# featureform/embeddinghub

Hardware: NVIDIA H100
Metric: k-NN queries/s (higher is better)
Workload: dtype f32

## Files before the change

embeddinghub_b200/csrc/walk.cuh:

```cuda
#pragma once
#include <cuda_bf16.h>

#include <type_traits>

#include "common.cuh"

namespace ehb {

struct GraphView {
  const float* vecs;
  const uint32_t* links0;
  const uint32_t* up_off;
  const uint32_t* links_up;
  const uint64_t* labels;
  const uint8_t* deleted;
  uint32_t n, dim, dpad, M, M0, entry;
  int32_t max_level;
  int32_t metric;
  const __nv_bfloat16* vecs16;
  const int8_t* codes8;
  const float4* terms8;
};

struct WalkCfg {
  uint32_t lcap;
  uint32_t hash_size;
  uint32_t G;
  uint32_t NG;
  uint32_t staged;
  uint32_t dense;
  uint32_t prefetch;
  uint32_t dcap;
};

constexpr uint32_t kMaxSinks = 16;
struct ResultSink {
  uint64_t* labels[kMaxSinks];
  float* dists[kMaxSinks];
  uint32_t* flags[kMaxSinks];
  uint32_t* slice_count;
  uint32_t n, qs, epoch;
  uint64_t* keys;
};

__host__ __device__ inline uint32_t align_up(uint32_t x, uint32_t a) { return (x + a - 1) / a * a; }

constexpr uint32_t kPadDims[] = {32, 64, 128, 256, 384, 512, 768, 1024, 1536, 2048};
constexpr uint32_t kNumPadDims = sizeof(kPadDims) / sizeof(kPadDims[0]);
__host__ __device__ constexpr int row_lpv(uint32_t row_bytes) { return row_bytes > 1024 ? 32 : 8; }
__host__ __device__ constexpr int row_nq(uint32_t dpad, uint32_t row_bytes) {
  return (int)(dpad / (4u * (uint32_t)row_lpv(row_bytes)));
}
constexpr int kpl_for(uint32_t ef) { return ef <= 64 ? 2 : (ef <= 128 ? 4 : (ef <= 256 ? 8 : 16)); }

inline uint32_t pad_dim(uint32_t dim) {
  for (uint32_t d : kPadDims)
    if (dim <= d) return d;
  return 0;
}

template <uint32_t MaxDpad = 2048, uint32_t I = 0, class F>
cudaError_t with_dpad(uint32_t dpad, F&& f) {
  if constexpr (I == kNumPadDims || kPadDims[I] > MaxDpad)
    return cudaErrorInvalidValue;
  else
    return dpad == kPadDims[I] ? f(std::integral_constant<uint32_t, kPadDims[I]>{})
                               : with_dpad<MaxDpad, I + 1>(dpad, f);
}

__host__ __device__ constexpr bool screen_shape(int LPV, int NQ) { return LPV == 32 && NQ <= 12; }

__host__ __device__ inline uint32_t warp_smem_bytes(const WalkCfg& c, uint32_t vbytes) {
  uint32_t b = 0;
  b += align_up(c.lcap * 8u, 128);
  b += align_up(c.hash_size * 4u, 128);
  b += 128;
  b += 128;
  b += 128;
  b += align_up(c.dcap * 8u, 128);
  b += c.staged ? align_up(c.G * c.NG * vbytes, 128) : 0u;
  return b;
}

struct WarpCtx {
  uint64_t* keys;
  uint32_t* hash;
  uint32_t* cand_id;
  float* cand_dist;
  uint64_t* mbar;
  uint32_t* dq_hi;
  uint32_t* dq_id;
  float* stage;
  uint32_t lcap, hsize, G, NG, dpad, vbytes, dcap, prefetch;
  uint32_t phases;
  uint32_t cnt;
  uint32_t lane;
};

__device__ __forceinline__ void ctx_init(WarpCtx& c, unsigned char* base, const WalkCfg& cfg, uint32_t dpad,
                                         uint32_t esize = 4u) {
  c.lane = lane_id();
  c.lcap = cfg.lcap;
  c.G = cfg.G;
  c.NG = cfg.NG;
  c.dpad = dpad;
  c.vbytes = dpad * esize;
  c.hsize = cfg.hash_size;
  unsigned char* p = base;
  c.keys = (uint64_t*)p;
  p += align_up(cfg.lcap * 8u, 128);
  c.hash = (uint32_t*)p;
  p += align_up(cfg.hash_size * 4u, 128);
  c.cand_id = (uint32_t*)p;
  p += 128;
  c.cand_dist = (float*)p;
  p += 128;
  c.mbar = (uint64_t*)p;
  p += 128;
  c.dcap = cfg.dcap;
  c.prefetch = cfg.prefetch;
  c.dq_hi = (uint32_t*)p;
  c.dq_id = c.dq_hi + cfg.dcap;
  p += align_up(cfg.dcap * 8u, 128);
  c.stage = (float*)p;
  c.phases = 0;
  c.cnt = 0;
  if (cfg.staged) {
    if (c.lane < cfg.NG) mbar_init(&c.mbar[c.lane], 1);
    fence_mbar_init();
  }
  __syncwarp();
}

__device__ __forceinline__ void hash_clear(WarpCtx& c) {
  uint4* h4 = (uint4*)c.hash;
  uint32_t n4 = c.hsize >> 2;
  for (uint32_t i = c.lane; i < n4; i += 32) h4[i] = make_uint4(kInvalid, kInvalid, kInvalid, kInvalid);
  __syncwarp();
}

__device__ __forceinline__ bool hash_insert(WarpCtx& c, uint32_t id, uint32_t& overflow) {
  uint32_t h = __umulhi(id * 0x9E3779B1u, c.hsize);
#pragma unroll 1
  for (int probe = 0; probe < 8; ++probe) {
    uint32_t old = atomicCAS(&c.hash[h], kInvalid, id);
    if (old == kInvalid) return true;
    if (old == id) return false;
    h = h + 1u == c.hsize ? 0u : h + 1u;
  }
  overflow = 1;
  return true;
}

template <class RowT, int NQ, int W = (std::is_same<RowT, __nv_bfloat16>::value && NQ > 1) ? 8 : 4>
struct LaneChunks {
  static_assert(W == 4 || (W == 8 && std::is_same<RowT, __nv_bfloat16>::value), "no such chunk");
  using T = std::conditional_t<std::is_same<RowT, float>::value, float4,
                               std::conditional_t<std::is_same<RowT, int8_t>::value, uint32_t,
                                                  std::conditional_t<W == 8, uint4, uint2>>>;
  static constexpr int V = W / 4;
  static constexpr int N = NQ / V;
};
__device__ __forceinline__ float4 ld_chunk(const float4* p) { return ld_nc_f4(p); }
__device__ __forceinline__ uint4 ld_chunk(const uint4* p) { return ld_nc_u4(p); }
__device__ __forceinline__ uint2 ld_chunk(const uint2* p) { return ld_nc_u2(p); }
__device__ __forceinline__ float4 bf16x4_to_f4(uint32_t a, uint32_t b) {
  return make_float4(__uint_as_float(a << 16), __uint_as_float(a & 0xFFFF0000u), __uint_as_float(b << 16),
                     __uint_as_float(b & 0xFFFF0000u));
}
__device__ __forceinline__ void widen(const float4& v, float4* x) { x[0] = v; }
__device__ __forceinline__ void widen(const uint4& v, float4* x) {
  x[0] = bf16x4_to_f4(v.x, v.y);
  x[1] = bf16x4_to_f4(v.z, v.w);
}
__device__ __forceinline__ void widen(const uint2& v, float4* x) { x[0] = bf16x4_to_f4(v.x, v.y); }
__device__ __forceinline__ void widen(const uint32_t& v, float4* x) {
  const uint32_t u = v ^ 0x80808080u;
  x[0] = make_float4(__uint_as_float(__byte_perm(u, 0x4B000000u, 0x7540)) - 8388736.0f,
                     __uint_as_float(__byte_perm(u, 0x4B000000u, 0x7541)) - 8388736.0f,
                     __uint_as_float(__byte_perm(u, 0x4B000000u, 0x7542)) - 8388736.0f,
                     __uint_as_float(__byte_perm(u, 0x4B000000u, 0x7543)) - 8388736.0f);
}

template <int LPV, int NQ, class RowT = float>
__device__ __forceinline__ void load_query_regs(float4 (&qr)[NQ], const float* __restrict__ src, uint32_t dim,
                                                uint32_t lane) {
  constexpr int V = LaneChunks<RowT, NQ>::V;
  uint32_t sub = lane % LPV;
#pragma unroll
  for (int t = 0; t < NQ; ++t) {
    uint32_t e = (sub + LPV * (t / V)) * 4u * V + 4u * (t % V);
    float4 v;
    v.x = e + 0 < dim ? src[e + 0] : 0.f;
    v.y = e + 1 < dim ? src[e + 1] : 0.f;
    v.z = e + 2 < dim ? src[e + 2] : 0.f;
    v.w = e + 3 < dim ? src[e + 3] : 0.f;
    qr[t] = v;
  }
}
template <int LPV, int NQ, class RowT, class C = LaneChunks<RowT, NQ>>
__device__ __forceinline__ void load_vec_regs(typename C::T (&r)[C::N], const RowT* __restrict__ row,
                                              uint32_t lane) {
  const typename C::T* p = (const typename C::T*)row + (lane % LPV);
#pragma unroll
  for (int t = 0; t < C::N; ++t) r[t] = p[LPV * t];
}

template <int NQ>
__device__ __forceinline__ float partial_dist(const float4 (&v)[NQ], const float4 (&qr)[NQ], int metric) {
  float a0 = 0.f, a1 = 0.f, a2 = 0.f, a3 = 0.f;
  if (metric == 0) {
#pragma unroll
    for (int t = 0; t < NQ; ++t) {
      float dx = qr[t].x - v[t].x, dy = qr[t].y - v[t].y, dz = qr[t].z - v[t].z, dw = qr[t].w - v[t].w;
      a0 = fmaf(dx, dx, a0);
      a1 = fmaf(dy, dy, a1);
      a2 = fmaf(dz, dz, a2);
      a3 = fmaf(dw, dw, a3);
    }
  } else {
#pragma unroll
    for (int t = 0; t < NQ; ++t) {
      a0 = fmaf(qr[t].x, v[t].x, a0);
      a1 = fmaf(qr[t].y, v[t].y, a1);
      a2 = fmaf(qr[t].z, v[t].z, a2);
      a3 = fmaf(qr[t].w, v[t].w, a3);
    }
  }
  return (a0 + a1) + (a2 + a3);
}
template <int LPV>
__device__ __forceinline__ float group_reduce(float acc) {
#pragma unroll
  for (int o = LPV / 2; o > 0; o >>= 1) acc += __shfl_xor_sync(0xffffffffu, acc, o);
  return acc;
}

template <int NQ, class RowT, class C = LaneChunks<RowT, NQ>>
__device__ __forceinline__ float chunk_dist(const typename C::T (&v)[C::N], const float4 (&qr)[NQ], int metric) {
  float4 x[NQ];
#pragma unroll
  for (int j = 0; j < C::N; ++j) widen(v[j], x + j * C::V);
  return partial_dist<NQ>(x, qr, metric);
}
template <class RowT>
__device__ __forceinline__ const RowT* walk_rows(const GraphView& g) {
  if constexpr (std::is_same<RowT, float>::value)
    return g.vecs;
  else
    return g.vecs16;
}

__host__ __device__ constexpr int eval_u(int N, int UDIV) {
  return ((N <= 2 ? 8 : (N <= 4 ? 4 : 2)) / UDIV) > 0 ? (N <= 2 ? 8 : (N <= 4 ? 4 : 2)) / UDIV : 1;
}
template <int NQ, int U = eval_u(NQ, 1), class RowT = float>
__device__ __forceinline__ void eval_direct(WarpCtx& c, const RowT* __restrict__ rows, const float4 (&qr)[NQ],
                                            uint32_t m, int metric) {
  using C = LaneChunks<RowT, NQ>;
  const uint32_t sub = c.lane & 7u, grp = c.lane >> 3;
  __syncwarp();
#pragma unroll 1
  for (uint32_t j0 = 0; j0 < m; j0 += 4 * U) {
    typename C::T v[U][C::N];
#pragma unroll
    for (int u = 0; u < U; ++u) {
      if (j0 + 4u * u < m) {
        uint32_t j = min(j0 + 4u * u + grp, m - 1u);
        const typename C::T* p = (const typename C::T*)(rows + (size_t)c.cand_id[j] * c.dpad) + sub;
#pragma unroll
        for (int t = 0; t < C::N; ++t) v[u][t] = ld_chunk(p + 8 * t);
      }
    }
#pragma unroll
    for (int u = 0; u < U; ++u) {
      if (j0 + 4u * u < m) {
        uint32_t j = j0 + 4u * u + grp;
        float acc = group_reduce<8>(chunk_dist<NQ, RowT>(v[u], qr, metric));
        if (sub == 0 && j < m) c.cand_dist[j] = metric == 0 ? acc : 1.0f - acc;
      }
    }
  }
  __syncwarp();
}

template <class RowT>
__device__ __forceinline__ void issue_rows(WarpCtx& c, const RowT* __restrict__ vecs, uint32_t r, uint32_t m,
                                           uint32_t G, uint32_t vbytes) {
  uint32_t buf = r % c.NG;
  uint32_t first = r * G;
  uint32_t cnt = min(G, m - first);
  if (c.lane == 0) mbar_arrive_expect_tx(&c.mbar[buf], cnt * vbytes);
  __syncwarp();
  if (c.lane < cnt) {
    uint32_t id = c.cand_id[first + c.lane];
    bulk_g2s((RowT*)c.stage + (size_t)(buf * G + c.lane) * c.dpad, vecs + (size_t)id * c.dpad, vbytes, &c.mbar[buf]);
  }
}
template <class RowT>
__device__ __forceinline__ void issue_group(WarpCtx& c, const RowT* __restrict__ vecs, uint32_t r, uint32_t m) {
  issue_rows(c, vecs, r, m, c.G, c.vbytes);
}
template <int NQ, class RowT>
__device__ __forceinline__ void eval_staged(WarpCtx& c, const RowT* __restrict__ vecs, const float4 (&qr)[NQ],
                                            uint32_t m, int metric) {
  const uint32_t rounds = (m + c.G - 1) / c.G;
  const uint32_t pre = min(rounds, c.NG);
  for (uint32_t r = 0; r < pre; ++r) issue_group(c, vecs, r, m);
#pragma unroll 1
  for (uint32_t r = 0; r < rounds; ++r) {
    uint32_t buf = r % c.NG;
    mbar_wait(&c.mbar[buf], (c.phases >> buf) & 1u);
    c.phases ^= (1u << buf);
    uint32_t first = r * c.G;
    uint32_t cnt = min(c.G, m - first);
#pragma unroll 1
    for (uint32_t v0 = 0; v0 < cnt; v0 += 4) {
      float acc[4];
#pragma unroll
      for (int i = 0; i < 4; ++i) {
        uint32_t v = min(v0 + (uint32_t)i, cnt - 1u);
        typename LaneChunks<RowT, NQ>::T x[LaneChunks<RowT, NQ>::N];
        load_vec_regs<32, NQ>(x, (const RowT*)c.stage + (size_t)(buf * c.G + v) * c.dpad, c.lane);
        acc[i] = chunk_dist<NQ, RowT>(x, qr, metric);
      }
#pragma unroll
      for (int o = 16; o > 0; o >>= 1) {
#pragma unroll
        for (int i = 0; i < 4; ++i) acc[i] += __shfl_xor_sync(0xffffffffu, acc[i], o);
      }
      if (c.lane < 4 && v0 + c.lane < cnt) {
        float a = c.lane == 0 ? acc[0] : (c.lane == 1 ? acc[1] : (c.lane == 2 ? acc[2] : acc[3]));
        c.cand_dist[first + v0 + c.lane] = metric == 0 ? a : 1.0f - a;
      }
    }
    __syncwarp();
    if (r + c.NG < rounds) {
      fence_proxy_async();
      issue_group(c, vecs, r + c.NG, m);
    }
  }
  __syncwarp();
}

template <int LPV, int NQ, int UDIV = 1, class RowT = float>
__device__ __forceinline__ void eval_candidates(WarpCtx& c, const RowT* __restrict__ vecs, const float4 (&qr)[NQ],
                                                uint32_t m, int metric) {
  if (LPV == 8)
    eval_direct<NQ, eval_u(LaneChunks<RowT, NQ>::N, UDIV)>(c, vecs, qr, m, metric);
  else
    eval_staged<NQ>(c, vecs, qr, m, metric);
}

struct ScreenQuery {
  float l1, l2, a;
};
__device__ __forceinline__ ScreenQuery* screen_query(const WarpCtx& c) { return (ScreenQuery*)(c.mbar + 8); }
template <int NQ>
__device__ __forceinline__ uint32_t screen_staged(WarpCtx& c, const GraphView& g, const float4 (&qr)[NQ], uint32_t m,
                                                  uint32_t worst_hi, uint32_t& unsure) {
  using C = LaneChunks<int8_t, NQ>;
  constexpr int SV = 4;
  const uint32_t G = min(4u * c.G, 32u), vbytes = c.dpad;
  const uint32_t rounds = (m + G - 1) / G;
  const uint32_t pre = min(rounds, c.NG);
  const bool in = c.lane < m;
  fence_proxy_async();
  for (uint32_t r = 0; r < pre; ++r) issue_rows(c, g.codes8, r, m, G, vbytes);
  if (in) prefetch_l2(g.terms8 + c.cand_id[c.lane]);
#pragma unroll 1
  for (uint32_t r = 0; r < rounds; ++r) {
    uint32_t buf = r % c.NG;
    mbar_wait(&c.mbar[buf], (c.phases >> buf) & 1u);
    c.phases ^= (1u << buf);
    uint32_t first = r * G;
    uint32_t cnt = min(G, m - first);
#pragma unroll 1
    for (uint32_t v0 = 0; v0 < cnt; v0 += SV) {
      float e[SV];
#pragma unroll
      for (int i = 0; i < SV; ++i) {
        uint32_t v = min(v0 + (uint32_t)i, cnt - 1u);
        const typename C::T* s4 = (const typename C::T*)((const int8_t*)c.stage + (size_t)(buf * G + v) * c.dpad) +
                                  c.lane;
        float4 x[NQ];
#pragma unroll
        for (int t = 0; t < C::N; ++t) widen(s4[32 * t], x + t);
        e[i] = partial_dist<NQ>(x, qr, 1);
      }
#pragma unroll
      for (int o = 16; o > 0; o >>= 1) {
#pragma unroll
        for (int i = 0; i < SV; ++i) e[i] += __shfl_xor_sync(0xffffffffu, e[i], o);
      }
      if (c.lane < (uint32_t)SV && v0 + c.lane < cnt) {
        float ea = e[0];
#pragma unroll
        for (int i = 1; i < SV; ++i)
          if (c.lane == (uint32_t)i) ea = e[i];
        c.cand_dist[first + v0 + c.lane] = ea;
      }
    }
    __syncwarp();
    if (r + c.NG < rounds) {
      fence_proxy_async();
      issue_rows(c, g.codes8, r + c.NG, m, G, vbytes);
    }
  }
  __syncwarp();
  float L = 0.f;
  const uint32_t id = in ? c.cand_id[c.lane] : kInvalid;
  if (in) {
    const float4 tm = ld_nc_f4(g.terms8 + id);
    const ScreenQuery sq = *screen_query(c);
    const float e = (float)c.dpad * 0x1p-24f;
    const float gam = __fdiv_ru(e, 1.0f - e), as = __fmul_ru((float)c.dpad, 0x1p-118f);
    const float se = __fmul_ru(tm.x, c.cand_dist[c.lane]);
    float mg = __fmul_ru(__fmul_ru(gam, sq.l2), __fmaf_ru(2.0f, tm.w, tm.z));
    mg = __fadd_ru(mg, fminf(__fmul_ru(sq.l1, tm.y), __fmul_ru(sq.l2, tm.z)));
    mg = __fadd_ru(mg, __fmaf_ru(tm.x, as, sq.a));
    L = __fsub_rd(__fsub_rd(1.0f, se), mg);
  }
  const bool keep = in && !(isfinite(L) && f2ord(L) >= worst_hi);
  const uint32_t mask = __ballot_sync(0xffffffffu, keep);
  const uint32_t pos = __popc(mask & lanemask_lt());
  __syncwarp();
  if (keep) c.cand_id[pos] = id;
  if (unsure) unsure = __reduce_or_sync(0xffffffffu, (keep && ((unsure >> c.lane) & 1u)) ? (1u << pos) : 0u);
  fence_proxy_async();
  __syncwarp();
  return __popc(mask);
}

template <int KPL>
struct UList {
  uint32_t hi[KPL];
  uint32_t id[KPL];
};
template <int KPL>
__device__ __forceinline__ void ul_clear(UList<KPL>& u, uint32_t ef, uint32_t lane) {
#pragma unroll
  for (int s = 0; s < KPL; ++s) {
    u.hi[s] = ((uint32_t)s * 32u + lane) < ef ? 0xFFFFFFFFu : 0u;
    u.id[s] = kInvalid;
  }
}
template <int KPL>
__device__ __forceinline__ uint32_t ul_worst(const UList<KPL>& u) {
  uint32_t m = u.hi[0];
#pragma unroll
  for (int s = 1; s < KPL; ++s) m = max(m, u.hi[s]);
  return __reduce_max_sync(0xffffffffu, m);
}
template <int KPL>
__device__ __forceinline__ void ul_insert(UList<KPL>& u, uint32_t hi, uint32_t id, uint32_t ef, uint32_t& cnt,
                                          uint32_t& worst_hi, uint32_t lane) {
  bool done = false;
  if (cnt < ef) {
#pragma unroll
    for (int s = 0; s < KPL; ++s) {
      if (!done) {
        uint32_t b = __ballot_sync(0xffffffffu, u.id[s] == kInvalid && u.hi[s] == 0xFFFFFFFFu);
        if (b) {
          if ((int)lane == __ffs(b) - 1) u.hi[s] = hi, u.id[s] = id;
          done = true;
        }
      }
    }
    cnt++;
    if (cnt == ef) worst_hi = ul_worst<KPL>(u);
  } else {
#pragma unroll
    for (int s = 0; s < KPL; ++s) {
      if (!done) {
        uint32_t b = __ballot_sync(0xffffffffu, u.hi[s] == worst_hi && u.id[s] != kInvalid);
        if (b) {
          if ((int)lane == __ffs(b) - 1) u.hi[s] = hi, u.id[s] = id;
          done = true;
        }
      }
    }
    worst_hi = ul_worst<KPL>(u);
  }
}
template <int KPL>
__device__ __forceinline__ uint32_t ul_min_unexpanded(UList<KPL>& u, bool mark, uint32_t lane) {
  uint32_t m = 0xFFFFFFFFu;
#pragma unroll
  for (int s = 0; s < KPL; ++s)
    if (!(u.id[s] & kExpandedFlag)) m = min(m, u.hi[s]);
  m = __reduce_min_sync(0xffffffffu, m);
  uint32_t node = kInvalid;
  bool done = false;
#pragma unroll
  for (int s = 0; s < KPL; ++s) {
    if (!done) {
      uint32_t b = __ballot_sync(0xffffffffu, !(u.id[s] & kExpandedFlag) && u.hi[s] == m);
      if (b) {
        int l = __ffs(b) - 1;
        node = __shfl_sync(0xffffffffu, u.id[s], l);
        if (mark && (int)lane == l) u.id[s] |= kExpandedFlag;
        done = true;
      }
    }
  }
  return node;
}
template <int KPL>
__device__ __forceinline__ uint32_t ul_min_unexpanded_hi(const UList<KPL>& u) {
  uint32_t m = 0xFFFFFFFFu;
#pragma unroll
  for (int s = 0; s < KPL; ++s)
    if (!(u.id[s] & kExpandedFlag)) m = min(m, u.hi[s]);
  return __reduce_min_sync(0xffffffffu, m);
}
template <int KPL>
__device__ __forceinline__ bool ul_contains(const UList<KPL>& u, uint32_t id) {
  bool hit = false;
#pragma unroll
  for (int s = 0; s < KPL; ++s) hit |= u.id[s] != kInvalid && (u.id[s] & kIdMask) == id;
  return __any_sync(0xffffffffu, hit);
}
template <int KPL>
__device__ __forceinline__ uint64_t ul_extract_min(UList<KPL>& u, uint32_t lane) {
  uint32_t m = 0xFFFFFFFFu;
#pragma unroll
  for (int s = 0; s < KPL; ++s)
    if (u.id[s] != kInvalid) m = min(m, u.hi[s]);
  m = __reduce_min_sync(0xffffffffu, m);
  uint64_t out = kMaxKey;
  bool done = false;
#pragma unroll
  for (int s = 0; s < KPL; ++s) {
    if (!done) {
      uint32_t b = __ballot_sync(0xffffffffu, u.id[s] != kInvalid && u.hi[s] == m);
      if (b) {
        int l = __ffs(b) - 1;
        uint32_t id = __shfl_sync(0xffffffffu, u.id[s], l);
        out = ((uint64_t)m << 32) | (id & kIdMask);
        if ((int)lane == l) u.id[s] = kInvalid, u.hi[s] = 0xFFFFFFFFu;
        done = true;
      }
    }
  }
  return out;
}
template <int KPL>
__device__ __forceinline__ void ul_extract_all(WarpCtx& c, UList<KPL>& u) {
  c.cnt = 0;
  for (;;) {
    uint64_t key = ul_extract_min<KPL>(u, c.lane);
    if (key == kMaxKey) break;
    if (c.lane == 0) c.keys[c.cnt] = key;
    c.cnt++;
  }
  __syncwarp();
}

__device__ __forceinline__ uint32_t list_insert(WarpCtx& c, uint64_t key, uint32_t limit) {
  const uint32_t id = key_id(key);
  uint32_t pos = 0;
  uint32_t dup = 0;
  for (uint32_t base = 0; base < c.cnt; base += 32) {
    uint32_t i = base + c.lane;
    uint64_t k = i < c.cnt ? c.keys[i] : kMaxKey;
    pos += __popc(__ballot_sync(0xffffffffu, k < key));
    dup |= __ballot_sync(0xffffffffu, i < c.cnt && key_id(k) == id);
  }
  if (dup || pos >= limit) return kInvalid;
  const uint32_t newcnt = min(c.cnt + 1u, limit);
  for (int base = (int)((newcnt - 1u) & ~31u); base >= (int)(pos & ~31u); base -= 32) {
    uint32_t i = (uint32_t)base + c.lane;
    bool in = i >= pos && i < newcnt;
    uint64_t v = key;
    if (in && i > pos) v = c.keys[i - 1];
    __syncwarp();
    if (in) c.keys[i] = v;
  }
  __syncwarp();
  c.cnt = newcnt;
  return pos;
}

struct WalkCounters {
  uint32_t hops_upper, hops_base, evals, overflow, screened, survivors;
};

__device__ __forceinline__ uint32_t load_row(const GraphView& g, uint32_t node, int level, uint32_t lane) {
  const uint32_t* row;
  uint32_t width;
  if (level == 0) {
    row = g.links0 + (size_t)node * g.M0;
    width = g.M0;
  } else {
    row = g.links_up + (size_t)(g.up_off[node] + (uint32_t)(level - 1)) * g.M;
    width = g.M;
  }
  uint32_t v = row[min(lane, width - 1u)];
  return lane < width ? v : kInvalid;
}

template <int LPV, int NQ, int UDIV = 1, class RowT = float>
__device__ __forceinline__ void greedy_descent(WarpCtx& c, const GraphView& g, const float4 (&qr)[NQ], uint32_t& cur,
                                               float& curdist, int from_level, int to_level_excl,
                                               WalkCounters& wc) {
  for (int level = from_level; level > to_level_excl; --level) {
    bool changed = true;
    while (changed) {
      changed = false;
      __syncwarp();
      uint32_t nb = load_row(g, cur, level, c.lane);
      uint32_t mask = __ballot_sync(0xffffffffu, nb != kInvalid);
      uint32_t m = __popc(mask);
      wc.hops_upper++;
      if (!m) break;
      if (nb != kInvalid) c.cand_id[__popc(mask & lanemask_lt())] = nb;
      __syncwarp();
      wc.evals += m;
      eval_candidates<LPV, NQ, UDIV>(c, walk_rows<RowT>(g), qr, m, g.metric);
      float bd = c.lane < m ? c.cand_dist[c.lane] : INFINITY;
      uint32_t bl = c.lane;
#pragma unroll
      for (int o = 16; o > 0; o >>= 1) {
        float od = __shfl_xor_sync(0xffffffffu, bd, o);
        uint32_t ol = __shfl_xor_sync(0xffffffffu, bl, o);
        if (od < bd || (od == bd && ol < bl)) bd = od, bl = ol;
      }
      if (bd < curdist) {
        curdist = bd;
        cur = c.cand_id[bl];
        changed = true;
      }
      __syncwarp();
    }
  }
}

__device__ __forceinline__ void dq_push(WarpCtx& c, uint32_t& dn, uint32_t hi, uint32_t id, uint32_t bound,
                                        uint32_t& overflow) {
  if (dn < c.dcap) {
    if (c.lane == 0) c.dq_hi[dn] = hi, c.dq_id[dn] = id;
    dn++;
  } else {
    uint32_t w = 0, wp = 0;
    for (uint32_t i = c.lane; i < dn; i += 32)
      if (c.dq_hi[i] >= w) w = c.dq_hi[i], wp = i;
    uint32_t wm = __reduce_max_sync(0xffffffffu, w);
    uint32_t b = __ballot_sync(0xffffffffu, w == wm);
    uint32_t pos = __shfl_sync(0xffffffffu, wp, __ffs(b) - 1);
    if (hi < wm && c.lane == 0) c.dq_hi[pos] = hi, c.dq_id[pos] = id;
    if (max(hi, wm) <= bound) overflow = 1;
  }
  __syncwarp();
}
__device__ __forceinline__ uint32_t dq_min(const WarpCtx& c, uint32_t dn, uint32_t& hi_out) {
  uint32_t m = 0xFFFFFFFFu, mp = kInvalid;
  for (uint32_t i = c.lane; i < dn; i += 32)
    if (c.dq_hi[i] < m) m = c.dq_hi[i], mp = i;
  uint32_t mm = __reduce_min_sync(0xffffffffu, m);
  uint32_t b = __ballot_sync(0xffffffffu, m == mm && mp != kInvalid);
  hi_out = mm;
  return b ? __shfl_sync(0xffffffffu, mp, __ffs(b) - 1) : kInvalid;
}

template <int LPV, int NQ, int KPL, bool PREFETCH, bool HASDEL, int UDIV = 1, class RowT = float>
__device__ __forceinline__ void beam_search(WarpCtx& c, const GraphView& g, const float4 (&qr)[NQ], UList<KPL>& u,
                                            uint32_t ep, float epdist, int level, uint32_t ef, uint32_t exclude,
                                            WalkCounters& wc) {
  constexpr bool kScreen = screen_shape(LPV, NQ) && std::is_same<RowT, float>::value;
  const bool screen = kScreen && g.codes8 && g.metric == 1;
  if (screen) {
    float mx = 0.f, l1 = 0.f, l2 = 0.f;
#pragma unroll
    for (int t = 0; t < NQ; ++t) {
      const float v[4] = {qr[t].x, qr[t].y, qr[t].z, qr[t].w};
#pragma unroll
      for (int j = 0; j < 4; ++j) {
        mx = fmaxf(mx, fabsf(v[j]));
        l1 = __fadd_ru(l1, fabsf(v[j]));
        l2 = __fmaf_ru(v[j], v[j], l2);
      }
    }
#pragma unroll
    for (int o = 16; o > 0; o >>= 1) {
      l1 = __fadd_ru(l1, __shfl_xor_sync(0xffffffffu, l1, o));
      l2 = __fadd_ru(l2, __shfl_xor_sync(0xffffffffu, l2, o));
    }
    mx = __uint_as_float(__reduce_max_sync(0xffffffffu, __float_as_uint(mx)));
    if (c.lane == 0)
      *screen_query(c) = {l1, __fsqrt_ru(l2), __fmul_ru((float)g.dpad, __fmaf_ru(mx, 0x1p-125f, 0x1p-124f))};
    __syncwarp();
  }
  hash_clear(c);
  ul_clear<KPL>(u, ef, c.lane);
  const uint8_t* __restrict__ del = (HASDEL && c.dcap) ? g.deleted : nullptr;
  uint32_t dn = 0;
  uint32_t ovf = 0;
  if (c.lane == 0) {
    hash_insert(c, ep, ovf);
    if (exclude != kInvalid) hash_insert(c, exclude, ovf);
  }
  __syncwarp();
  uint32_t cnt = 0;
  uint32_t worst_hi = 0xFFFFFFFFu;
  bool ovf_any = false;
  const bool ep_result = ep != exclude && !(del && del[ep]);
  if (ep_result) ul_insert<KPL>(u, f2ord(epdist), ep, ef, cnt, worst_hi, c.lane);
  uint32_t node = ep;
  if (ep_result) node = ul_min_unexpanded<KPL>(u, true, c.lane);
  uint32_t nb = load_row(g, node, level, c.lane);
  for (;;) {
    if (level == 0) wc.hops_base++; else wc.hops_upper++;
    if (HASDEL && wc.hops_base + wc.hops_upper > 64u * ef + 65536u) break;
    __syncwarp();
    const uint32_t spec = ul_min_unexpanded<KPL>(u, false, c.lane);
    uint32_t spec_row = kInvalid;
    if (spec != kInvalid) spec_row = load_row(g, spec & kIdMask, level, c.lane);
    bool is_new = false;
    uint32_t o = 0;
    if (nb != kInvalid && nb != exclude) is_new = hash_insert(c, nb, o);
    ovf |= o;
    __syncwarp();
    uint32_t mask = __ballot_sync(0xffffffffu, is_new);
    uint32_t m = __popc(mask);
    if (m) {
      const uint32_t pos = __popc(mask & lanemask_lt());
      if (is_new) c.cand_id[pos] = nb;
      uint32_t unsure = (HASDEL && del) ? __reduce_or_sync(0xffffffffu, (is_new && o) ? (1u << pos) : 0u) : 0u;
      __syncwarp();
      wc.evals += m;
      if (kScreen && screen && cnt >= ef) {
        wc.screened += m;
        m = screen_staged<NQ>(c, g, qr, m, worst_hi, unsure);
        wc.survivors += m;
      }
      eval_candidates<LPV, NQ, UDIV>(c, walk_rows<RowT>(g), qr, m, g.metric);
      if (PREFETCH && LPV == 8 && c.prefetch && spec_row != kInvalid) {
        const char* pv = (const char*)(walk_rows<RowT>(g) + (size_t)spec_row * g.dpad);
#pragma unroll
        for (int b = 0; b < NQ * 8 * 16 * (int)sizeof(RowT) / 4; b += 128) prefetch_l2(pv + b);
      }
      uint32_t myhi = 0xFFFFFFFFu, myid = kInvalid;
      if (c.lane < m) myhi = f2ord(c.cand_dist[c.lane]), myid = c.cand_id[c.lane];
      const bool mydel = HASDEL && del && c.lane < m && del[myid];
      __syncwarp();
      ovf_any = ovf_any || __any_sync(0xffffffffu, ovf);
      uint32_t qual = __ballot_sync(0xffffffffu, c.lane < m && (cnt < ef || myhi < worst_hi));
      const uint32_t delmask = (HASDEL && del) ? __ballot_sync(0xffffffffu, mydel) : 0u;
      while (qual) {
        int j = __ffs(qual) - 1;
        qual &= qual - 1;
        uint32_t hj = __shfl_sync(0xffffffffu, myhi, j);
        uint32_t ij = __shfl_sync(0xffffffffu, myid, j);
        if (cnt >= ef && hj >= worst_hi) continue;
        if (HASDEL && ((delmask >> j) & 1u)) {
          if (!((unsure >> j) & 1u)) dq_push(c, dn, hj, ij, cnt >= ef ? worst_hi : 0xFFFFFFFFu, ovf);
          continue;
        }
        if (ovf_any && ul_contains<KPL>(u, ij)) continue;
        ul_insert<KPL>(u, hj, ij, ef, cnt, worst_hi, c.lane);
        if (PREFETCH && c.lane == 0) prefetch_l2(g.links0 + (size_t)ij * g.M0);
      }
    }
    if (HASDEL && dn) {
      uint32_t dhi;
      const uint32_t dpos = dq_min(c, dn, dhi);
      if (dhi < ul_min_unexpanded_hi<KPL>(u)) {
        if (cnt >= ef && dhi > worst_hi) break;
        node = c.dq_id[dpos];
        __syncwarp();
        if (c.lane == 0) c.dq_hi[dpos] = c.dq_hi[dn - 1], c.dq_id[dpos] = c.dq_id[dn - 1];
        dn--;
        __syncwarp();
        nb = load_row(g, node, level, c.lane);
        continue;
      }
    }
    node = ul_min_unexpanded<KPL>(u, true, c.lane);
    if (node == kInvalid) break;
    nb = (node == spec) ? spec_row : load_row(g, node, level, c.lane);
  }
  wc.overflow |= (ovf_any || __any_sync(0xffffffffu, ovf)) ? 1u : 0u;
}

}
```

Before: 440,800.

## Load screen terms early and evaluate survivors with direct batched fp32 loads

The per-candidate screening terms are now loaded into registers before the staged int8 loop instead of only being prefetched to L2, which hides their latency behind the screening work. After screening, survivors are evaluated by a new routine that loads fp32 rows straight from global memory in register batches, bypassing the staged asynchronous copy path. This avoids the setup and synchronisation overhead of staging for the few survivors, at the cost of more registers and a hardcoded inner-product distance (1 - dot) that ignores the metric argument.

Measured after the change: 458,900 (median of 6 runs). 4.1% higher.

```diff
diff --git a/embeddinghub_b200/csrc/walk.cuh b/embeddinghub_b200/csrc/walk.cuh
--- a/embeddinghub_b200/csrc/walk.cuh
+++ b/embeddinghub_b200/csrc/walk.cuh
@@ -367,7 +367,9 @@
   const bool in = c.lane < m;
   fence_proxy_async();
   for (uint32_t r = 0; r < pre; ++r) issue_rows(c, g.codes8, r, m, G, vbytes);
-  if (in) prefetch_l2(g.terms8 + c.cand_id[c.lane]);
+  const uint32_t id = in ? c.cand_id[c.lane] : kInvalid;
+  float4 tm = make_float4(0.f, 0.f, 0.f, 0.f);
+  if (in) tm = ld_nc_f4(g.terms8 + id);
 #pragma unroll 1
   for (uint32_t r = 0; r < rounds; ++r) {
     uint32_t buf = r % c.NG;
@@ -409,9 +411,7 @@
   }
   __syncwarp();
   float L = 0.f;
-  const uint32_t id = in ? c.cand_id[c.lane] : kInvalid;
   if (in) {
-    const float4 tm = ld_nc_f4(g.terms8 + id);
     const ScreenQuery sq = *screen_query(c);
     const float e = (float)c.dpad * 0x1p-24f;
     const float gam = __fdiv_ru(e, 1.0f - e), as = __fmul_ru((float)c.dpad, 0x1p-118f);
@@ -430,6 +430,39 @@
   fence_proxy_async();
   __syncwarp();
   return __popc(mask);
+}
+
+template <int NQ>
+__device__ __forceinline__ void eval_survivors(WarpCtx& c, const float* __restrict__ vecs, const float4 (&qr)[NQ],
+                                               uint32_t m) {
+  constexpr int SB = NQ <= 24 ? 24 / NQ : 1;
+#pragma unroll 1
+  for (uint32_t v0 = 0; v0 < m; v0 += SB) {
+    float4 x[SB][NQ];
+#pragma unroll
+    for (int i = 0; i < SB; ++i) {
+      const uint32_t v = min(v0 + (uint32_t)i, m - 1u);
+      const float4* p = (const float4*)(vecs + (size_t)c.cand_id[v] * c.dpad) + c.lane;
+#pragma unroll
+      for (int t = 0; t < NQ; ++t) x[i][t] = ld_nc_f4(p + 32 * t);
+    }
+    float acc[SB];
+#pragma unroll
+    for (int i = 0; i < SB; ++i) acc[i] = chunk_dist<NQ, float>(x[i], qr, 1);
+#pragma unroll
+    for (int o = 16; o > 0; o >>= 1) {
+#pragma unroll
+      for (int i = 0; i < SB; ++i) acc[i] += __shfl_xor_sync(0xffffffffu, acc[i], o);
+    }
+    if (c.lane < (uint32_t)SB && v0 + c.lane < m) {
+      float a = acc[0];
+#pragma unroll
+      for (int i = 1; i < SB; ++i)
+        if (c.lane == (uint32_t)i) a = acc[i];
+      c.cand_dist[v0 + c.lane] = 1.0f - a;
+    }
+  }
+  __syncwarp();
 }
 
 template <int KPL>
@@ -733,8 +766,10 @@
         wc.screened += m;
         m = screen_staged<NQ>(c, g, qr, m, worst_hi, unsure);
         wc.survivors += m;
-      }
-      eval_candidates<LPV, NQ, UDIV>(c, walk_rows<RowT>(g), qr, m, g.metric);
+        eval_survivors<NQ>(c, g.vecs, qr, m);
+      } else {
+        eval_candidates<LPV, NQ, UDIV>(c, walk_rows<RowT>(g), qr, m, g.metric);
+      }
       if (PREFETCH && LPV == 8 && c.prefetch && spec_row != kInvalid) {
         const char* pv = (const char*)(walk_rows<RowT>(g) + (size_t)spec_row * g.dpad);
 #pragma unroll
```
